# PierfrancescoArdino/C2M

Hardware: AMD Instinct MI355X
Metric: generator train-step frames/sec at 128x256x7 (higher is better)
Workload: dtype f32; 1 GPU; BASELINE configs[1]: 128x256, 7-frame clips (2 in + 5 predicted), batch 8/GPU, fp32, generator fwd+bwd only (no D), VGG loss on, random-init weights; global_batch=8, parallelism=single

## Files before the change

c2m_amd/csrc/conv_wino4.hip:

```cpp
#include "common.h"
#include <stdlib.h>

typedef float f32x16 __attribute__((ext_vector_type(16)));
typedef float f32x4 __attribute__((ext_vector_type(4)));
typedef float f32x2 __attribute__((ext_vector_type(2)));
typedef unsigned u32x4 __attribute__((ext_vector_type(4)));
#define W4_OOB 0x80000000u

struct Wino4P {
    const float* U;
    const float* X;
    float* Y;
    const float* bias;
    float* Y2;
    long y2_sn, y2_sc, y2_sh;
    int lo_y, lo_x, ext_y, ext_x;
    int M, K, nimg;
    int Hi, Wi, Ho, Wo;
    int iy0, ix0;
    int reflect;
    long in_sn, out_sn, out_sc, out_sh, out_off;
    int in_sc, in_sh;
    unsigned x_bytes;
    int nchunks, mtiles;
    int act;
    float slope;
    const float* R;
    int r_l;
};

#if !defined(W4_SKEW) && !defined(W4_FUSED)
#define W4_FUSED 1
#endif

constexpr int W4_CK = 8;
constexpr int W4_TH = 4, W4_TW = 8;
constexpr int W4_OR = 4 * W4_TH, W4_OC = 4 * W4_TW;
constexpr int W4_PH = W4_OR + 2, W4_PW = W4_OC + 2;
constexpr int W4_PITCH = 40;
constexpr int W4_PPOS = W4_PH * W4_PITCH;
constexpr int W4_ROWS = (W4_PPOS + 63) / 64;
constexpr int W4_PCS = 722;
constexpr int W4_PBUF = W4_CK * W4_PCS + 48;
constexpr int W4_TAB = W4_ROWS * 64;
constexpr int W4_VBUF = 36 * W4_CK * 32;

#define W4_BT(o0, o1, o2, o3, o4, o5, x0, x1, x2, x3, x4, x5) \
    do {                                                      \
        const float a_ = (x4) - 2.25f * (x2), b_ = 0.75f * (x3) - 1.6875f * (x1);          \
        const float c_ = (x4) - 0.5625f * (x2), e_ = 1.5f * (x3) - 0.84375f * (x1);        \
        o0 = 1.265625f * (x0) - 2.8125f * (x2) + (x4);        \
        o1 = a_ + b_; o2 = a_ - b_; o3 = c_ + e_; o4 = c_ - e_; \
        o5 = 1.265625f * (x1) - 2.8125f * (x3) + (x5);        \
    } while (0)

#ifdef W4_TRACE
__device__ unsigned long long w4_trace_buf[8 * 16 * 4 + 8 * 2];
#define W4_STAMP(i) do { if (blockIdx.x == 0 && lane == 0 && n < 16) sTr[(wave * 16 + n) * 4 + (i)] = clock64(); } while (0)
C2M_API int c2m_wino4_trace_read(unsigned long long* host) {
    return (int)hipMemcpyFromSymbol(host, HIP_SYMBOL(w4_trace_buf), sizeof(w4_trace_buf));
}
#else
#define W4_STAMP(i) do { } while (0)
#endif

__global__ __launch_bounds__(512, 2) void conv_wino4_kernel(const Wino4P p) {
    __shared__ __attribute__((aligned(16))) float smem[3 * W4_PBUF + W4_TAB + 2 * W4_VBUF];
#ifdef W4_TRACE
    __shared__ unsigned long long sTr[8 * 16 * 4 + 8 * 2];
    const unsigned long long t_begin = clock64();
#endif
#define sP (smem)
#define sVo (reinterpret_cast<unsigned*>(smem + 3 * W4_PBUF))
#define sV (smem + 3 * W4_PBUF + W4_TAB)
    const int tid = threadIdx.x, lane = tid & 63;
    const int wave = __builtin_amdgcn_readfirstlane(tid >> 6);
    const int wm = wave & 1, fg = wave >> 1;
    const bool t_first = (wave ^ (wave >> 2)) & 1;
    const int regions_x = (p.Wo + W4_OC - 1) / W4_OC, regions_y = (p.Ho + W4_OR - 1) / W4_OR;
    int rb, mt;
    {
        const unsigned L = blockIdx.x, total = gridDim.x;
        const unsigned q = total >> 3, r = total & 7u, x = L & 7u, j = L >> 3;
        const unsigned w = x * q + (x < r ? x : r) + j;
        mt = (int)(w % (unsigned)p.mtiles); rb = (int)(w / (unsigned)p.mtiles);
    }
    const int rx = rb % regions_x; rb /= regions_x;
    const int ry = rb % regions_y; const int img = rb / regions_y;
    const int oy0 = ry * W4_OR, ox0 = rx * W4_OC;
    const int nchunks = p.nchunks;

    {
        const unsigned img_byte = (unsigned)(img * (int)p.in_sn) * 4u;
        for (int pos = tid; pos < W4_TAB; pos += 512) {
            const int r = pos / W4_PITCH, c = pos % W4_PITCH;
            int iy = oy0 + p.iy0 + r, ix = ox0 + p.ix0 + c;
            if (p.reflect) {
                iy = iy < 0 ? -iy : iy; iy = iy >= p.Hi ? 2 * p.Hi - 2 - iy : iy;
                ix = ix < 0 ? -ix : ix; ix = ix >= p.Wi ? 2 * p.Wi - 2 - ix : ix;
            }
            const bool ok = pos < W4_PPOS && c < W4_PW && (unsigned)iy < (unsigned)p.Hi && (unsigned)ix < (unsigned)p.Wi;
            sVo[pos] = ok ? img_byte + (unsigned)(iy * p.in_sh + ix) * 4u : W4_OOB;
        }
    }
    __syncthreads();

    const unsigned long xaddr = (unsigned long)p.X;
    const u32x4 rs = {(unsigned)xaddr, (unsigned)(xaddr >> 32) & 0xffffu, p.x_bytes, 0x00020000u};
    const unsigned sp_lds = (unsigned)(unsigned long)(__attribute__((address_space(3))) float*)&smem[0];
    unsigned pvo[W4_ROWS];
#pragma unroll
    for (int dr = 0; dr < W4_ROWS; ++dr) pvo[dr] = sVo[dr * 64 + lane];
    auto load_patch = [&](int chunk, int buf, const int dr0 = 0, const int dr1 = W4_ROWS) __attribute__((always_inline)) {
#ifdef W4_ZERO_RECORDS
        const int ch = chunk * W4_CK + wave;
        u32x4 rsk = rs;
        rsk[2] = (chunk < nchunks && ch < p.K) ? p.x_bytes : 0u;
#else
        int ch = chunk * W4_CK + wave;
        ch = ch < p.K ? ch : p.K - 1;
        const u32x4 rsk = rs;
#endif
        const int soff = ch * p.in_sc * 4;
#pragma unroll
        for (int dr = dr0; dr < dr1; ++dr) {
            const unsigned vo = pvo[dr];
            const unsigned dst = sp_lds + (unsigned)((buf * W4_PBUF + wave * W4_PCS + dr * 64) * 4);
            if (dr * 64 + 64 <= W4_PPOS || dr * 64 + lane < W4_PPOS)
                asm volatile("s_mov_b32 m0, %0\n\ts_nop 0\n\tbuffer_load_dword %1, %2, %3 offen lds"
                             :: "s"(dst), "v"(vo), "s"(rsk), "s"(soff) : "memory");
        }
    };
    const unsigned long uaddr = (unsigned long)p.U;
    const u32x4 urs = {(unsigned)uaddr, (unsigned)(uaddr >> 32) & 0xffffu, 0xffffffffu, 0x00020000u};
    const unsigned uvo = (unsigned)((((mt * 8 + wave) * 9) * 64 + lane) * 16);
    const unsigned ustride_b = (unsigned)p.mtiles * 8u * 9u * 64u * 16u;
    f32x4 ua[9];
    auto load_u = [&](int chunk) __attribute__((always_inline)) {
        const int s0 = (int)((unsigned)(chunk < nchunks ? chunk : 0) * ustride_b), s1 = s0 + 4096, s2 = s0 + 8192;
#pragma unroll
        for (int f = 0; f < 9; ++f)
            asm volatile("buffer_load_dwordx4 %0, %1, %2, %3 offen offset:%4"
                         : "=&v"(ua[f]) : "v"(uvo), "s"(urs), "s"(f < 4 ? s0 : (f < 8 ? s1 : s2)), "n"((f & 3) * 1024) : "memory");
    };

    f32x16 acc[9];
#pragma unroll
    for (int f = 0; f < 9; ++f)
#pragma unroll
        for (int r = 0; r < 16; ++r) acc[f][r] = 0.f;

    const int item = tid & 255, th = __builtin_amdgcn_readfirstlane(tid >> 8);
    const int tk = item >> 5, tn = item & 31;
    const int pbase = tk * W4_PCS + (4 * (tn >> 3)) * W4_PITCH + 4 * (tn & 7);
    auto transform = [&](int pb, int vb) __attribute__((always_inline)) {
        const float* __restrict__ src = sP + pb * W4_PBUF + pbase;
        float t[3][6];
#pragma unroll
        for (int cp = 0; cp < 3; ++cp) {
            f32x2 d[6];
#pragma unroll
            for (int r = 0; r < 6; ++r) d[r] = *reinterpret_cast<const f32x2*>(src + r * W4_PITCH + 2 * cp);
#pragma unroll
            for (int e = 0; e < 2; ++e) {
                const float d0 = d[0][e], d1 = d[1][e], d2 = d[2][e], d3 = d[3][e], d4 = d[4][e], d5 = d[5][e];
                const int c = 2 * cp + e;
                if (th == 0) {
                    const float a_ = d4 - 2.25f * d2, b_ = 0.75f * d3 - 1.6875f * d1;
                    t[0][c] = 1.265625f * d0 - 2.8125f * d2 + d4; t[1][c] = a_ + b_; t[2][c] = a_ - b_;
                } else {
                    const float c_ = d4 - 0.5625f * d2, e_ = 1.5f * d3 - 0.84375f * d1;
                    t[0][c] = c_ + e_; t[1][c] = c_ - e_; t[2][c] = 1.265625f * d1 - 2.8125f * d3 + d5;
                }
            }
        }
        float* __restrict__ v = sV + vb * W4_VBUF + tk * 32 + tn;
#pragma unroll
        for (int a = 0; a < 3; ++a) {
            float o0, o1, o2, o3, o4, o5;
            W4_BT(o0, o1, o2, o3, o4, o5, t[a][0], t[a][1], t[a][2], t[a][3], t[a][4], t[a][5]);
            const int xi0 = 6 * (3 * th + a);
            v[(xi0 + 0) * W4_CK * 32] = o0; v[(xi0 + 1) * W4_CK * 32] = o1; v[(xi0 + 2) * W4_CK * 32] = o2;
            v[(xi0 + 3) * W4_CK * 32] = o3; v[(xi0 + 4) * W4_CK * 32] = o4; v[(xi0 + 5) * W4_CK * 32] = o5;
            __builtin_amdgcn_sched_barrier(0);
        }
    };
    auto mma = [&](int cur, int next_chunk) __attribute__((always_inline)) {
        const float* __restrict__ vb = sV + cur * W4_VBUF + (9 * fg * W4_CK + (lane >> 5)) * 32 + (lane & 31);
        const int s0 = (int)((unsigned)(next_chunk < nchunks ? next_chunk : 0) * ustride_b), s1 = s0 + 4096, s2 = s0 + 8192;
#pragma unroll
        for (int g3 = 0; g3 < 3; ++g3) {
            float b[3][4];
#pragma unroll
            for (int f = 0; f < 3; ++f)
#pragma unroll
                for (int kk = 0; kk < 4; ++kk) b[f][kk] = vb[((3 * g3 + f) * W4_CK + 2 * kk) * 32];
#pragma unroll
            for (int kk = 0; kk < 4; ++kk)
#pragma unroll
                for (int f = 0; f < 3; ++f) {
                    const f32x4 u = ua[3 * g3 + f];
                    const float av = kk == 0 ? u.x : (kk == 1 ? u.y : (kk == 2 ? u.z : u.w));
                    acc[3 * g3 + f] = __builtin_amdgcn_mfma_f32_32x32x2f32(av, b[f][kk], acc[3 * g3 + f], 0, 0, 0);
                }
            __builtin_amdgcn_sched_barrier(0);
#pragma unroll
            for (int f = 3 * g3; f < 3 * g3 + 3; ++f)
                asm volatile("buffer_load_dwordx4 %0, %1, %2, %3 offen offset:%4"
                             : "=&v"(ua[f]) : "v"(uvo), "s"(urs), "s"(f < 4 ? s0 : (f < 8 ? s1 : s2)), "n"((f & 3) * 1024) : "memory");
            __builtin_amdgcn_sched_barrier(0);
        }
    };

#ifdef W4_FUSED
    const float cA = th ? 0.5625f : 2.25f, cB3 = th ? 1.5f : 0.75f, cB1 = th ? 0.84375f : 1.6875f;
    const int xrow = th ? 5 : 0, r_single = th ? 5 : 0, r_plus = th ? 3 : 1, r_minus = th ? 4 : 2;
    auto fused = [&](int cur, int next_chunk, int pb, int dbuf) __attribute__((always_inline)) {
        const float* __restrict__ vb = sV + cur * W4_VBUF + (9 * fg * W4_CK + (lane >> 5)) * 32 + (lane & 31);
        const float* __restrict__ src = sP + pb * W4_PBUF + pbase;
        const int s0 = (int)((unsigned)(next_chunk < nchunks ? next_chunk : 0) * ustride_b), s1 = s0 + 4096, s2 = s0 + 8192;
        float ts[6], tp[6], tm[6];
        float b[3][4];
        f32x2 d1, d2, d3, d4, dx;
        auto reads = [&](const int g3) __attribute__((always_inline)) {
#pragma unroll
            for (int f = 0; f < 3; ++f)
#pragma unroll
                for (int kk = 0; kk < 4; ++kk) b[f][kk] = vb[((3 * g3 + f) * W4_CK + 2 * kk) * 32];
            d1 = *reinterpret_cast<const f32x2*>(src + 1 * W4_PITCH + 2 * g3); d2 = *reinterpret_cast<const f32x2*>(src + 2 * W4_PITCH + 2 * g3);
            d3 = *reinterpret_cast<const f32x2*>(src + 3 * W4_PITCH + 2 * g3); d4 = *reinterpret_cast<const f32x2*>(src + 4 * W4_PITCH + 2 * g3);
            dx = *reinterpret_cast<const f32x2*>(src + xrow * W4_PITCH + 2 * g3);
        };
        asm volatile("s_waitcnt vmcnt(12)" ::: "memory");
#pragma unroll
        for (int f = 0; f < 3; ++f) asm volatile("" : "+v"(ua[f]));
        reads(0);
#pragma unroll
        for (int g3 = 0; g3 < 3; ++g3) {
#pragma unroll
            for (int kk = 0; kk < 4; ++kk)
#pragma unroll
                for (int f = 0; f < 3; ++f) {
                    const f32x4 u = ua[3 * g3 + f];
                    const float av = kk == 0 ? u.x : (kk == 1 ? u.y : (kk == 2 ? u.z : u.w));
                    acc[3 * g3 + f] = __builtin_amdgcn_mfma_f32_32x32x2f32(av, b[f][kk], acc[3 * g3 + f], 0, 0, 0);
                }
#pragma unroll
            for (int e = 0; e < 2; ++e) {
                const int c = 2 * g3 + e;
                const float q0 = th ? d1[e] : dx[e], q2 = th ? d3[e] : d2[e], q4 = th ? dx[e] : d4[e];
                ts[c] = 1.265625f * q0 - 2.8125f * q2 + q4;
                const float a_ = d4[e] - cA * d2[e], b_ = cB3 * d3[e] - cB1 * d1[e];
                tp[c] = a_ + b_; tm[c] = a_ - b_;
            }
            if (g3 == 0) __builtin_amdgcn_sched_group_barrier(0x100, 17, 0);
#pragma unroll
            for (int q = 0; q < 12; ++q) {
                __builtin_amdgcn_sched_group_barrier(0x008, 1, 0);
                __builtin_amdgcn_sched_group_barrier(0x002, 2, 0);
            }
            __builtin_amdgcn_sched_barrier(0);
            if (g3 < 2) reads(g3 + 1);
            if (g3 < 2) load_patch(next_chunk + 1, dbuf, 6 * g3, 6 * g3 + 6);
#pragma unroll
            for (int f = 3 * g3; f < 3 * g3 + 3; ++f)
                asm volatile("buffer_load_dwordx4 %0, %1, %2, %3 offen offset:%4"
                             : "=&v"(ua[f]) : "v"(uvo), "s"(urs), "s"(f < 4 ? s0 : (f < 8 ? s1 : s2)), "n"((f & 3) * 1024) : "memory");
            if (g3 == 0) asm volatile("s_waitcnt vmcnt(12)" ::: "memory");
            if (g3 == 1) asm volatile("s_waitcnt vmcnt(18)" ::: "memory");
            if (g3 < 2) {
#pragma unroll
                for (int f = 3 * g3 + 3; f < 3 * g3 + 6; ++f) asm volatile("" : "+v"(ua[f]));
            }
            __builtin_amdgcn_sched_barrier(0);
        }
        float* __restrict__ v = sV + (cur ^ 1) * W4_VBUF + tk * 32 + tn;
#pragma unroll
        for (int a = 0; a < 3; ++a) {
            const float* t = a == 0 ? ts : (a == 1 ? tp : tm);
            const int row = a == 0 ? r_single : (a == 1 ? r_plus : r_minus);
            float o0, o1, o2, o3, o4, o5;
            W4_BT(o0, o1, o2, o3, o4, o5, t[0], t[1], t[2], t[3], t[4], t[5]);
            float* __restrict__ vr = v + 6 * row * W4_CK * 32;
            vr[0] = o0; vr[1 * W4_CK * 32] = o1; vr[2 * W4_CK * 32] = o2;
            vr[3 * W4_CK * 32] = o3; vr[4 * W4_CK * 32] = o4; vr[5 * W4_CK * 32] = o5;
        }
    };
#endif

    load_patch(0, 0);
    load_patch(1, 1);
    load_u(0);
    asm volatile("s_waitcnt vmcnt(21)" ::: "memory");
    __syncthreads();
    transform(0, 0);
#ifdef W4_FUSED
    asm volatile("s_waitcnt vmcnt(0)" ::: "memory");
#else
    asm volatile("s_waitcnt vmcnt(9)" ::: "memory");
#endif
    int pn = 1;
#ifdef W4_PRIO
    if (wave >= 4) __builtin_amdgcn_s_setprio(1);
#endif
    for (int n = 0; n < nchunks; ++n) {
        __syncthreads();
        W4_STAMP(0);
        const int cur = n & 1;
        const int dbuf = pn == 2 ? 0 : pn + 1;
#ifndef W4_FUSED
        load_patch(n + 2, dbuf);
#endif
        __builtin_amdgcn_sched_barrier(0);
#ifdef W4_FUSED
        W4_STAMP(1);
        fused(cur, n + 1, pn, dbuf);
        W4_STAMP(2);
        W4_STAMP(3);
#else
        if (t_first) transform(pn, cur ^ 1);
        asm volatile("s_waitcnt vmcnt(12)" ::: "memory");
#pragma unroll
        for (int f = 0; f < 9; ++f) asm volatile("" : "+v"(ua[f]));
        W4_STAMP(1);
        mma(cur, n + 1);
        W4_STAMP(2);
        if (!t_first) transform(pn, cur ^ 1);
        W4_STAMP(3);
#endif
#ifdef W4_FUSED
        asm volatile("s_waitcnt vmcnt(6)" ::: "memory");
#else
        asm volatile("s_waitcnt vmcnt(9)" ::: "memory");
#endif
        pn = pn == 2 ? 0 : pn + 1;
    }
    asm volatile("s_waitcnt vmcnt(0)" ::: "memory");
#pragma unroll
    for (int f = 0; f < 9; ++f) asm volatile("" :: "v"(ua[f]));
    __syncthreads();

    float* __restrict__ sR = sV;
    const int etile = tid & 31, ecl = tid >> 5;
    const int ety = etile >> 3, etx = etile & 7;
    const int oyb = oy0 + 4 * ety, oxb = ox0 + 4 * etx;
    float bias4[4];
#pragma unroll
    for (int pass = 0; pass < 4; ++pass) {
        const int co = mt * 64 + (pass >> 1) * 32 + (pass & 1) * 16 + ecl;
        bias4[pass] = (p.bias && co < p.M) ? p.bias[co] : 0.f;
    }
#pragma unroll
    for (int pass = 0; pass < 4; ++pass) {
        const int pwm = pass >> 1, hf = pass & 1;
        __syncthreads();
        if (wm == pwm) {
#pragma unroll
            for (int f = 0; f < 9; ++f)
#pragma unroll
                for (int rr = 0; rr < 8; ++rr) {
                    const int rowl = (rr & 3) + 8 * (rr >> 2) + 4 * (lane >> 5);
                    sR[((9 * fg + f) * 16 + rowl) * 32 + (lane & 31)] = hf ? acc[f][8 + rr] : acc[f][rr];
                }
        }
        __syncthreads();
        const int cout = mt * 64 + pwm * 32 + hf * 16 + ecl;
        float y[4][4];
        {
            float s[6][4];
#pragma unroll
            for (int i = 0; i < 6; ++i) {
                const float* __restrict__ q = sR + ((6 * i) * 16 + ecl) * 32 + etile;
                const float m0 = q[0], m1 = q[16 * 32], m2 = q[2 * 16 * 32], m3 = q[3 * 16 * 32], m4 = q[4 * 16 * 32], m5 = q[5 * 16 * 32];
                const float pp = m1 + m2, nn = m1 - m2, PP = m3 + m4, NN = m3 - m4;
                s[i][0] = m0 + pp + PP; s[i][1] = 0.75f * nn + 1.5f * NN; s[i][2] = 0.5625f * pp + 2.25f * PP;
                s[i][3] = 0.421875f * nn + 3.375f * NN + m5;
            }
#pragma unroll
            for (int c = 0; c < 4; ++c) {
                const float pp = s[1][c] + s[2][c], nn = s[1][c] - s[2][c], PP = s[3][c] + s[4][c], NN = s[3][c] - s[4][c];
                y[0][c] = s[0][c] + pp + PP; y[1][c] = 0.75f * nn + 1.5f * NN; y[2][c] = 0.5625f * pp + 2.25f * PP;
                y[3][c] = 0.421875f * nn + 3.375f * NN + s[5][c];
            }
        }
        if (cout < p.M) {
            const float bb = bias4[pass];
            const float* __restrict__ rb = p.R ? p.R + ((long)img * p.M + cout) * 4 * p.r_l : nullptr;
#pragma unroll
            for (int r = 0; r < 4; ++r) {
                const int oy = oyb + r;
                if (oy >= p.Ho) continue;
                if (rb) {
                    if (oy == 1 || oy == p.Ho - 2) {
                        const float* __restrict__ rr = rb + (oy == 1 ? 0 : p.r_l) + oxb;
#pragma unroll
                        for (int c = 0; c < 4; ++c) if (oxb + c < p.Wo) y[r][c] += rr[c];
                    }
                    if (oxb <= 1 && oxb + 3 >= 1) {
                        const float v = rb[2 * p.r_l + oy];
#pragma unroll
                        for (int c = 0; c < 4; ++c) if (oxb + c == 1) y[r][c] += v;
                    }
                    if (oxb <= p.Wo - 2 && oxb + 3 >= p.Wo - 2) {
                        const float v = rb[3 * p.r_l + oy];
#pragma unroll
                        for (int c = 0; c < 4; ++c) if (oxb + c == p.Wo - 2) y[r][c] += v;
                    }
                }
                if (p.act == C2M_ACT_NONE) {
#pragma unroll
                    for (int c = 0; c < 4; ++c) y[r][c] += bb;
                } else if (p.act == C2M_ACT_LRELU) {
#pragma unroll
                    for (int c = 0; c < 4; ++c) { const float v = y[r][c] + bb; y[r][c] = v > 0.f ? v : p.slope * v; }
                } else {
#pragma unroll
                    for (int c = 0; c < 4; ++c) y[r][c] = c2m_act(y[r][c] + bb, p.act, p.slope);
                }
                float* __restrict__ yb0 = p.Y + p.out_off + (long)img * p.out_sn + (long)cout * p.out_sc + (long)oy * p.out_sh + oxb;
                typedef float f32x4u __attribute__((ext_vector_type(4), aligned(4)));
                const f32x4u vv = {y[r][0], y[r][1], y[r][2], y[r][3]};
                const int yi = oy - p.lo_y, xi0 = oxb - p.lo_x;
                const bool row_in = p.Y2 && (unsigned)yi < (unsigned)p.ext_y;
                const bool all_in = row_in && xi0 >= 0 && xi0 + 3 < p.ext_x;
                const bool all_out = !row_in || xi0 + 3 < 0 || xi0 >= p.ext_x;
                if (oxb + 3 < p.Wo && (!p.Y2 || all_out)) {
                    *reinterpret_cast<f32x4u*>(yb0) = vv;
                } else if (oxb + 3 < p.Wo && all_in) {
                    *reinterpret_cast<f32x4u*>(p.Y2 + (long)img * p.y2_sn + (long)cout * p.y2_sc + (long)yi * p.y2_sh + xi0) = vv;
                } else {
#pragma unroll
                    for (int c = 0; c < 4; ++c) {
                        if (oxb + c >= p.Wo) continue;
                        const int xi = oxb + c - p.lo_x;
                        if (row_in && (unsigned)xi < (unsigned)p.ext_x)
                            p.Y2[(long)img * p.y2_sn + (long)cout * p.y2_sc + (long)yi * p.y2_sh + xi] = y[r][c];
                        else
                            yb0[c] = y[r][c];
                    }
                }
            }
        }
    }
#ifdef W4_TRACE
    if (blockIdx.x == 0 && lane == 0) { sTr[8 * 16 * 4 + wave * 2] = t_begin; sTr[8 * 16 * 4 + wave * 2 + 1] = clock64(); }
    __syncthreads();
    if (blockIdx.x == 0)
        for (int i = tid; i < 8 * 16 * 4 + 8 * 2; i += 512) w4_trace_buf[i] = sTr[i];
#endif
}

#undef sP
#undef sVo
#undef sV

__global__ void wino4_filter_kernel(const float* __restrict__ w, float* __restrict__ up, int M, int K, int Cin_native,
                                    int dgrad, int mtiles, long pairs) {
    for (long i = blockIdx.x * (long)blockDim.x + threadIdx.x; i < pairs; i += (long)gridDim.x * blockDim.x) {
        const int kk = (int)(i & 3); long r = i >> 2;
        const int lane = (int)(r & 63); r >>= 6;
        const int wm = (int)(r & 1); r >>= 1;
        const int mt = (int)(r % mtiles); const int chunk = (int)(r / mtiles);
        const int m = mt * 64 + wm * 32 + (lane & 31), c = chunk * W4_CK + 2 * kk + (lane >> 5);
        float u[6][6];
#pragma unroll
        for (int a = 0; a < 6; ++a)
#pragma unroll
            for (int b2 = 0; b2 < 6; ++b2) u[a][b2] = 0.f;
        if (m < M && c < K) {
            const float* __restrict__ g = dgrad ? w + ((long)c * Cin_native + m) * 9 : w + ((long)m * Cin_native + c) * 9;
            float gg[3][3];
#pragma unroll
            for (int a = 0; a < 3; ++a)
#pragma unroll
                for (int b2 = 0; b2 < 3; ++b2) gg[a][b2] = dgrad ? g[(2 - a) * 3 + (2 - b2)] : g[a * 3 + b2];
            float row[6][3];
#pragma unroll
            for (int b2 = 0; b2 < 3; ++b2) {
                const float g0 = gg[0][b2], g1 = gg[1][b2], g2 = gg[2][b2];
                row[0][b2] = (64.f / 81.f) * g0;
                row[1][b2] = -(128.f / 243.f) * g0 - (32.f / 81.f) * g1 - (8.f / 27.f) * g2;
                row[2][b2] = -(128.f / 243.f) * g0 + (32.f / 81.f) * g1 - (8.f / 27.f) * g2;
                row[3][b2] = (32.f / 243.f) * g0 + (16.f / 81.f) * g1 + (8.f / 27.f) * g2;
                row[4][b2] = (32.f / 243.f) * g0 - (16.f / 81.f) * g1 + (8.f / 27.f) * g2;
                row[5][b2] = g2;
            }
#pragma unroll
            for (int a = 0; a < 6; ++a) {
                const float r0 = row[a][0], r1 = row[a][1], r2 = row[a][2];
                u[a][0] = (64.f / 81.f) * r0;
                u[a][1] = -(128.f / 243.f) * r0 - (32.f / 81.f) * r1 - (8.f / 27.f) * r2;
                u[a][2] = -(128.f / 243.f) * r0 + (32.f / 81.f) * r1 - (8.f / 27.f) * r2;
                u[a][3] = (32.f / 243.f) * r0 + (16.f / 81.f) * r1 + (8.f / 27.f) * r2;
                u[a][4] = (32.f / 243.f) * r0 - (16.f / 81.f) * r1 + (8.f / 27.f) * r2;
                u[a][5] = r2;
            }
        }
        const long base = ((long)chunk * mtiles + mt) * 8;
#pragma unroll
        for (int a = 0; a < 6; ++a)
#pragma unroll
            for (int b2 = 0; b2 < 6; ++b2) {
                const int xi = 6 * a + b2, fgi = xi / 9, f = xi % 9;
                up[((((base + ((fgi << 1) | wm)) * 9 + f) * 64 + lane) << 2) + kk] = u[a][b2];
            }
    }
}

C2M_API long c2m_wino4_upack_floats(int M, int K) {
    return 36L * (c2m_cdiv(M, 64) * 64L) * (c2m_cdiv(K, W4_CK) * (long)W4_CK);
}

C2M_API int c2m_wino4_filter_transform(const float* w, float* upack, int Cout, int Cin, int dgrad, void* stream) {
    C2M_ENTER();
    const int M = dgrad ? Cin : Cout, K = dgrad ? Cout : Cin;
    if (M <= 0 || K <= 0) return 0;
    const long total = c2m_wino4_upack_floats(M, K);
    if (total * 4 >= 0xffffffffL) return (int)hipErrorInvalidValue;
    hipLaunchKernelGGL(wino4_filter_kernel, dim3(c2m_grid(total / 36, 256)), dim3(256), 0, (hipStream_t)stream, w, upack, M,
                       K, Cin, dgrad, c2m_cdiv(M, 64), total / 36);
    return (int)hipGetLastError();
}

C2M_API int c2m_wino4_regions(int Ho, int Wo) { return c2m_cdiv(Ho, W4_OR) * c2m_cdiv(Wo, W4_OC); }

C2M_API int c2m_conv_wino4(const float* upack, const float* X, float* Y, float* Y_interior, const float* bias,
                           const int64_t* g, int act, float slope, void* stream) {
    C2M_ENTER();
    Wino4P p;
    p.U = upack; p.X = X; p.Y = Y; p.bias = bias;
    p.Y2 = Y_interior; p.y2_sn = p.y2_sc = p.y2_sh = 0; p.lo_y = p.lo_x = p.ext_y = p.ext_x = 0;
    if (Y_interior) {
        p.y2_sn = g[C2M_WG_Y2_SN]; p.y2_sc = g[C2M_WG_Y2_SC]; p.y2_sh = g[C2M_WG_Y2_SH];
        p.lo_y = (int)g[C2M_WG_LO_Y]; p.lo_x = (int)g[C2M_WG_LO_X]; p.ext_y = (int)g[C2M_WG_EXT_Y]; p.ext_x = (int)g[C2M_WG_EXT_X];
    }
    p.M = (int)g[C2M_WG_M]; p.K = (int)g[C2M_WG_K]; p.nimg = (int)g[C2M_WG_NIMG];
    p.Hi = (int)g[C2M_WG_HI]; p.Wi = (int)g[C2M_WG_WI]; p.Ho = (int)g[C2M_WG_HO]; p.Wo = (int)g[C2M_WG_WO];
    p.iy0 = (int)g[C2M_WG_IY0]; p.ix0 = (int)g[C2M_WG_IX0]; p.reflect = (int)g[C2M_WG_REFLECT];
    p.in_sn = g[C2M_WG_IN_SN]; p.in_sc = (int)g[C2M_WG_IN_SC]; p.in_sh = (int)g[C2M_WG_IN_SH];
    p.out_sn = g[C2M_WG_OUT_SN]; p.out_sc = g[C2M_WG_OUT_SC]; p.out_sh = g[C2M_WG_OUT_SH]; p.out_off = g[C2M_WG_OUT_OFF];
    if (g[C2M_WG_X_BYTES] <= 0 || g[C2M_WG_X_BYTES] >= 0x80000000LL) return (int)hipErrorInvalidValue;
    p.x_bytes = (unsigned)g[C2M_WG_X_BYTES];
    if (g[C2M_WG_NKT] != 0 || g[C2M_WG_PTAB] != 0) return (int)hipErrorInvalidValue;
    p.R = (const float*)(uintptr_t)g[C2M_WG_RING]; p.r_l = (int)g[C2M_WG_RING_L];
    if (p.R && (Y_interior || p.reflect || p.Ho < 4 || p.Wo < 4 || p.r_l < p.Ho || p.r_l < p.Wo || p.out_off != 0)) return (int)hipErrorInvalidValue;
    p.act = act; p.slope = slope;
    if (p.M <= 0 || p.K <= 0 || p.nimg <= 0 || p.Ho <= 0 || p.Wo <= 0) return 0;
    if ((((uintptr_t)upack) & 15) != 0) return (int)hipErrorInvalidValue;
    p.nchunks = c2m_cdiv(p.K, W4_CK);
    p.mtiles = c2m_cdiv(p.M, 64);
    if (c2m_wino4_upack_floats(p.M, p.K) * 4 >= 0xffffffffL) return (int)hipErrorInvalidValue;
    const long regions = (long)p.nimg * c2m_wino4_regions(p.Ho, p.Wo);
    if (regions * p.mtiles > 0x7fffffffL) return (int)hipErrorInvalidValue;
    hipLaunchKernelGGL(conv_wino4_kernel, dim3((unsigned)(regions * p.mtiles)), dim3(512), 0, (hipStream_t)stream, p);
    return (int)hipGetLastError();
}
```

Measured before the change: 892.9 frames/s.

## Make Winograd conv kernel persistent with cross-tile prefetch overlapping epilogue

```diff
diff --git a/c2m_amd/csrc/conv_wino4.hip b/c2m_amd/csrc/conv_wino4.hip
--- a/c2m_amd/csrc/conv_wino4.hip
+++ b/c2m_amd/csrc/conv_wino4.hip
@@ -23,6 +23,7 @@
     int in_sc, in_sh;
     unsigned x_bytes;
     int nchunks, mtiles;
+    unsigned items;
     int act;
     float slope;
     const float* R;
@@ -56,7 +57,7 @@
 
 #ifdef W4_TRACE
 __device__ unsigned long long w4_trace_buf[8 * 16 * 4 + 8 * 2];
-#define W4_STAMP(i) do { if (blockIdx.x == 0 && lane == 0 && n < 16) sTr[(wave * 16 + n) * 4 + (i)] = clock64(); } while (0)
+#define W4_STAMP(i) do { if (blockIdx.x == 0 && lane == 0 && n < 16 && it == it_first) sTr[(wave * 16 + n) * 4 + (i)] = clock64(); } while (0)
 C2M_API int c2m_wino4_trace_read(unsigned long long* host) {
     return (int)hipMemcpyFromSymbol(host, HIP_SYMBOL(w4_trace_buf), sizeof(w4_trace_buf));
 }
@@ -65,7 +66,7 @@
 #endif
 
 __global__ __launch_bounds__(512, 2) void conv_wino4_kernel(const Wino4P p) {
-    __shared__ __attribute__((aligned(16))) float smem[3 * W4_PBUF + W4_TAB + 2 * W4_VBUF];
+    __shared__ __attribute__((aligned(16))) float smem[3 * W4_PBUF + W4_TAB + 2 * W4_VBUF + 64];
 #ifdef W4_TRACE
     __shared__ unsigned long long sTr[8 * 16 * 4 + 8 * 2];
     const unsigned long long t_begin = clock64();
@@ -73,28 +74,42 @@
 #define sP (smem)
 #define sVo (reinterpret_cast<unsigned*>(smem + 3 * W4_PBUF))
 #define sV (smem + 3 * W4_PBUF + W4_TAB)
+#define sBias (smem + 3 * W4_PBUF + W4_TAB + 2 * W4_VBUF)
     const int tid = threadIdx.x, lane = tid & 63;
     const int wave = __builtin_amdgcn_readfirstlane(tid >> 6);
     const int wm = wave & 1, fg = wave >> 1;
     const bool t_first = (wave ^ (wave >> 2)) & 1;
     const int regions_x = (p.Wo + W4_OC - 1) / W4_OC, regions_y = (p.Ho + W4_OR - 1) / W4_OR;
-    int rb, mt;
+    unsigned it, it_end;
     {
-        const unsigned L = blockIdx.x, total = gridDim.x;
-        const unsigned q = total >> 3, r = total & 7u, x = L & 7u, j = L >> 3;
-        const unsigned w = x * q + (x < r ? x : r) + j;
-        mt = (int)(w % (unsigned)p.mtiles); rb = (int)(w / (unsigned)p.mtiles);
+        const unsigned L = blockIdx.x, G = gridDim.x;
+        const unsigned q = p.items >> 3, r = p.items & 7u, x = L & 7u, j = L >> 3;
+        const unsigned sx = x * q + (x < r ? x : r), cx = q + (x < r ? 1u : 0u);
+        const unsigned gx = (G >> 3) + (x < (G & 7u) ? 1u : 0u);
+        it = sx + (unsigned)((unsigned long)j * cx / gx);
+        it_end = sx + (unsigned)((unsigned long)(j + 1) * cx / gx);
     }
-    const int rx = rb % regions_x; rb /= regions_x;
-    const int ry = rb % regions_y; const int img = rb / regions_y;
-    const int oy0 = ry * W4_OR, ox0 = rx * W4_OC;
+    if (it >= it_end) return;
+#ifdef W4_TRACE
+    const unsigned it_first = it;
+#endif
+    struct Item { int mt, rb, img, oy0, ox0; };
+    auto decode = [&](unsigned w) __attribute__((always_inline)) {
+        Item d;
+        d.mt = (int)(w % (unsigned)p.mtiles); d.rb = (int)(w / (unsigned)p.mtiles);
+        const int rx = d.rb % regions_x, t = d.rb / regions_x;
+        d.img = t / regions_y;
+        d.oy0 = (t % regions_y) * W4_OR; d.ox0 = rx * W4_OC;
+        return d;
+    };
+    Item cur_it = decode(it);
     const int nchunks = p.nchunks;
 
-    {
-        const unsigned img_byte = (unsigned)(img * (int)p.in_sn) * 4u;
+    auto build_table = [&](const Item& d) __attribute__((always_inline)) {
+        const unsigned img_byte = (unsigned)(d.img * (int)p.in_sn) * 4u;
         for (int pos = tid; pos < W4_TAB; pos += 512) {
             const int r = pos / W4_PITCH, c = pos % W4_PITCH;
-            int iy = oy0 + p.iy0 + r, ix = ox0 + p.ix0 + c;
+            int iy = d.oy0 + p.iy0 + r, ix = d.ox0 + p.ix0 + c;
             if (p.reflect) {
                 iy = iy < 0 ? -iy : iy; iy = iy >= p.Hi ? 2 * p.Hi - 2 - iy : iy;
                 ix = ix < 0 ? -ix : ix; ix = ix >= p.Wi ? 2 * p.Wi - 2 - ix : ix;
@@ -102,15 +117,23 @@
             const bool ok = pos < W4_PPOS && c < W4_PW && (unsigned)iy < (unsigned)p.Hi && (unsigned)ix < (unsigned)p.Wi;
             sVo[pos] = ok ? img_byte + (unsigned)(iy * p.in_sh + ix) * 4u : W4_OOB;
         }
-    }
+    };
+    auto stage_bias = [&](int mt_) __attribute__((always_inline)) {
+        if (tid < 64) { const int co = mt_ * 64 + tid; sBias[tid] = (p.bias && co < p.M) ? p.bias[co] : 0.f; }
+    };
+    build_table(cur_it);
+    stage_bias(cur_it.mt);
     __syncthreads();
 
     const unsigned long xaddr = (unsigned long)p.X;
     const u32x4 rs = {(unsigned)xaddr, (unsigned)(xaddr >> 32) & 0xffffu, p.x_bytes, 0x00020000u};
     const unsigned sp_lds = (unsigned)(unsigned long)(__attribute__((address_space(3))) float*)&smem[0];
     unsigned pvo[W4_ROWS];
-#pragma unroll
-    for (int dr = 0; dr < W4_ROWS; ++dr) pvo[dr] = sVo[dr * 64 + lane];
+    auto read_pvo = [&]() __attribute__((always_inline)) {
+#pragma unroll
+        for (int dr = 0; dr < W4_ROWS; ++dr) pvo[dr] = sVo[dr * 64 + lane];
+    };
+    read_pvo();
     auto load_patch = [&](int chunk, int buf, const int dr0 = 0, const int dr1 = W4_ROWS) __attribute__((always_inline)) {
 #ifdef W4_ZERO_RECORDS
         const int ch = chunk * W4_CK + wave;
@@ -133,7 +156,7 @@
     };
     const unsigned long uaddr = (unsigned long)p.U;
     const u32x4 urs = {(unsigned)uaddr, (unsigned)(uaddr >> 32) & 0xffffu, 0xffffffffu, 0x00020000u};
-    const unsigned uvo = (unsigned)((((mt * 8 + wave) * 9) * 64 + lane) * 16);
+    unsigned uvo = (unsigned)((((cur_it.mt * 8 + wave) * 9) * 64 + lane) * 16);
     const unsigned ustride_b = (unsigned)p.mtiles * 8u * 9u * 64u * 16u;
     f32x4 ua[9];
     auto load_u = [&](int chunk) __attribute__((always_inline)) {
@@ -145,10 +168,6 @@
     };
 
     f32x16 acc[9];
-#pragma unroll
-    for (int f = 0; f < 9; ++f)
-#pragma unroll
-        for (int r = 0; r < 16; ++r) acc[f][r] = 0.f;
 
     const int item = tid & 255, th = __builtin_amdgcn_readfirstlane(tid >> 8);
     const int tk = item >> 5, tn = item & 31;
@@ -299,10 +318,16 @@
 #else
     asm volatile("s_waitcnt vmcnt(9)" ::: "memory");
 #endif
-    int pn = 1;
 #ifdef W4_PRIO
     if (wave >= 4) __builtin_amdgcn_s_setprio(1);
 #endif
+    for (;;) {
+    const int mt = cur_it.mt, img = cur_it.img, oy0 = cur_it.oy0, ox0 = cur_it.ox0;
+#pragma unroll
+    for (int f = 0; f < 9; ++f)
+#pragma unroll
+        for (int r = 0; r < 16; ++r) acc[f][r] = 0.f;
+    int pn = 1;
     for (int n = 0; n < nchunks; ++n) {
         __syncthreads();
         W4_STAMP(0);
@@ -340,16 +365,29 @@
     for (int f = 0; f < 9; ++f) asm volatile("" :: "v"(ua[f]));
     __syncthreads();
 
+    const bool more = it + 1 < it_end;
+    Item nxt = cur_it;
+    if (more) {
+        nxt = decode(it + 1);
+        if (nxt.rb != cur_it.rb) {
+            build_table(nxt);
+            __syncthreads();
+            read_pvo();
+        }
+        load_patch(0, 0);
+        load_patch(1, 1);
+    }
+
     float* __restrict__ sR = sV;
-    const int etile = tid & 31, ecl = tid >> 5;
+    const Wino4P& pe = p;
+    int etid = tid;
+    asm volatile("" : "+v"(etid));
+    const int etile = etid & 31, ecl = etid >> 5;
     const int ety = etile >> 3, etx = etile & 7;
     const int oyb = oy0 + 4 * ety, oxb = ox0 + 4 * etx;
     float bias4[4];
 #pragma unroll
-    for (int pass = 0; pass < 4; ++pass) {
-        const int co = mt * 64 + (pass >> 1) * 32 + (pass & 1) * 16 + ecl;
-        bias4[pass] = (p.bias && co < p.M) ? p.bias[co] : 0.f;
-    }
+    for (int pass = 0; pass < 4; ++pass) bias4[pass] = sBias[(pass >> 1) * 32 + (pass & 1) * 16 + ecl];
 #pragma unroll
     for (int pass = 0; pass < 4; ++pass) {
         const int pwm = pass >> 1, hf = pass & 1;
@@ -364,6 +402,11 @@
                 }
         }
         __syncthreads();
+        if (pass == 3 && more) {
+            uvo = (unsigned)((((nxt.mt * 8 + wave) * 9) * 64 + lane) * 16);
+            stage_bias(nxt.mt);
+            load_u(0);
+        }
         const int cout = mt * 64 + pwm * 32 + hf * 16 + ecl;
         float y[4][4];
         {
@@ -383,64 +426,75 @@
                 y[3][c] = 0.421875f * nn + 3.375f * NN + s[5][c];
             }
         }
-        if (cout < p.M) {
+        if (pass == 3 && more) {
+            asm volatile("s_waitcnt vmcnt(0)" ::: "memory");
+#pragma unroll
+            for (int f = 0; f < 9; ++f) asm volatile("" : "+v"(ua[f]));
+            __syncthreads();
+            read_pvo();
+            transform(0, 0);
+        }
+        if (cout < pe.M) {
             const float bb = bias4[pass];
-            const float* __restrict__ rb = p.R ? p.R + ((long)img * p.M + cout) * 4 * p.r_l : nullptr;
+            const float* __restrict__ rb = pe.R ? pe.R + ((long)img * pe.M + cout) * 4 * pe.r_l : nullptr;
 #pragma unroll
             for (int r = 0; r < 4; ++r) {
                 const int oy = oyb + r;
-                if (oy >= p.Ho) continue;
+                if (oy >= pe.Ho) continue;
                 if (rb) {
-                    if (oy == 1 || oy == p.Ho - 2) {
-                        const float* __restrict__ rr = rb + (oy == 1 ? 0 : p.r_l) + oxb;
-#pragma unroll
-                        for (int c = 0; c < 4; ++c) if (oxb + c < p.Wo) y[r][c] += rr[c];
+                    if (oy == 1 || oy == pe.Ho - 2) {
+                        const float* __restrict__ rr = rb + (oy == 1 ? 0 : pe.r_l) + oxb;
+#pragma unroll
+                        for (int c = 0; c < 4; ++c) if (oxb + c < pe.Wo) y[r][c] += rr[c];
                     }
                     if (oxb <= 1 && oxb + 3 >= 1) {
-                        const float v = rb[2 * p.r_l + oy];
+                        const float v = rb[2 * pe.r_l + oy];
 #pragma unroll
                         for (int c = 0; c < 4; ++c) if (oxb + c == 1) y[r][c] += v;
                     }
-                    if (oxb <= p.Wo - 2 && oxb + 3 >= p.Wo - 2) {
-                        const float v = rb[3 * p.r_l + oy];
-#pragma unroll
-                        for (int c = 0; c < 4; ++c) if (oxb + c == p.Wo - 2) y[r][c] += v;
+                    if (oxb <= pe.Wo - 2 && oxb + 3 >= pe.Wo - 2) {
+                        const float v = rb[3 * pe.r_l + oy];
+#pragma unroll
+                        for (int c = 0; c < 4; ++c) if (oxb + c == pe.Wo - 2) y[r][c] += v;
                     }
                 }
-                if (p.act == C2M_ACT_NONE) {
+                if (pe.act == C2M_ACT_NONE) {
 #pragma unroll
                     for (int c = 0; c < 4; ++c) y[r][c] += bb;
-                } else if (p.act == C2M_ACT_LRELU) {
-#pragma unroll
-                    for (int c = 0; c < 4; ++c) { const float v = y[r][c] + bb; y[r][c] = v > 0.f ? v : p.slope * v; }
+                } else if (pe.act == C2M_ACT_LRELU) {
+#pragma unroll
+                    for (int c = 0; c < 4; ++c) { const float v = y[r][c] + bb; y[r][c] = v > 0.f ? v : pe.slope * v; }
                 } else {
 #pragma unroll
-                    for (int c = 0; c < 4; ++c) y[r][c] = c2m_act(y[r][c] + bb, p.act, p.slope);
+                    for (int c = 0; c < 4; ++c) y[r][c] = c2m_act(y[r][c] + bb, pe.act, pe.slope);
                 }
-                float* __restrict__ yb0 = p.Y + p.out_off + (long)img * p.out_sn + (long)cout * p.out_sc + (long)oy * p.out_sh + oxb;
+                float* __restrict__ yb0 = pe.Y + pe.out_off + (long)img * pe.out_sn + (long)cout * pe.out_sc + (long)oy * pe.out_sh + oxb;
                 typedef float f32x4u __attribute__((ext_vector_type(4), aligned(4)));
                 const f32x4u vv = {y[r][0], y[r][1], y[r][2], y[r][3]};
-                const int yi = oy - p.lo_y, xi0 = oxb - p.lo_x;
-                const bool row_in = p.Y2 && (unsigned)yi < (unsigned)p.ext_y;
-                const bool all_in = row_in && xi0 >= 0 && xi0 + 3 < p.ext_x;
-                const bool all_out = !row_in || xi0 + 3 < 0 || xi0 >= p.ext_x;
-                if (oxb + 3 < p.Wo && (!p.Y2 || all_out)) {
+                const int yi = oy - pe.lo_y, xi0 = oxb - pe.lo_x;
+                const bool row_in = pe.Y2 && (unsigned)yi < (unsigned)pe.ext_y;
+                const bool all_in = row_in && xi0 >= 0 && xi0 + 3 < pe.ext_x;
+                const bool all_out = !row_in || xi0 + 3 < 0 || xi0 >= pe.ext_x;
+                if (oxb + 3 < pe.Wo && (!pe.Y2 || all_out)) {
                     *reinterpret_cast<f32x4u*>(yb0) = vv;
-                } else if (oxb + 3 < p.Wo && all_in) {
-                    *reinterpret_cast<f32x4u*>(p.Y2 + (long)img * p.y2_sn + (long)cout * p.y2_sc + (long)yi * p.y2_sh + xi0) = vv;
+                } else if (oxb + 3 < pe.Wo && all_in) {
+                    *reinterpret_cast<f32x4u*>(pe.Y2 + (long)img * pe.y2_sn + (long)cout * pe.y2_sc + (long)yi * pe.y2_sh + xi0) = vv;
                 } else {
 #pragma unroll
                     for (int c = 0; c < 4; ++c) {
-                        if (oxb + c >= p.Wo) continue;
-                        const int xi = oxb + c - p.lo_x;
-                        if (row_in && (unsigned)xi < (unsigned)p.ext_x)
-                            p.Y2[(long)img * p.y2_sn + (long)cout * p.y2_sc + (long)yi * p.y2_sh + xi] = y[r][c];
+                        if (oxb + c >= pe.Wo) continue;
+                        const int xi = oxb + c - pe.lo_x;
+                        if (row_in && (unsigned)xi < (unsigned)pe.ext_x)
+                            pe.Y2[(long)img * pe.y2_sn + (long)cout * pe.y2_sc + (long)yi * pe.y2_sh + xi] = y[r][c];
                         else
                             yb0[c] = y[r][c];
                     }
                 }
             }
         }
+    }
+    if (!more) break;
+    cur_it = nxt; ++it;
     }
 #ifdef W4_TRACE
     if (blockIdx.x == 0 && lane == 0) { sTr[8 * 16 * 4 + wave * 2] = t_begin; sTr[8 * 16 * 4 + wave * 2 + 1] = clock64(); }
@@ -453,6 +507,7 @@
 #undef sP
 #undef sVo
 #undef sV
+#undef sBias
 
 __global__ void wino4_filter_kernel(const float* __restrict__ w, float* __restrict__ up, int M, int K, int Cin_native,
                                     int dgrad, int mtiles, long pairs) {
@@ -523,6 +578,17 @@
 }
 
 C2M_API int c2m_wino4_regions(int Ho, int Wo) { return c2m_cdiv(Ho, W4_OR) * c2m_cdiv(Wo, W4_OC); }
+
+static int wino4_cu_count() {
+    static int cached[64];
+    int dev = 0;
+    if (hipGetDevice(&dev) != hipSuccess || dev < 0) return 0;
+    if (dev < 64 && cached[dev] > 0) return cached[dev];
+    int n = 0;
+    if (hipDeviceGetAttribute(&n, hipDeviceAttributeMultiprocessorCount, dev) != hipSuccess) return 0;
+    if (dev < 64) cached[dev] = n;
+    return n;
+}
 
 C2M_API int c2m_conv_wino4(const float* upack, const float* X, float* Y, float* Y_interior, const float* bias,
                            const int64_t* g, int act, float slope, void* stream) {
@@ -552,6 +618,10 @@
     if (c2m_wino4_upack_floats(p.M, p.K) * 4 >= 0xffffffffL) return (int)hipErrorInvalidValue;
     const long regions = (long)p.nimg * c2m_wino4_regions(p.Ho, p.Wo);
     if (regions * p.mtiles > 0x7fffffffL) return (int)hipErrorInvalidValue;
-    hipLaunchKernelGGL(conv_wino4_kernel, dim3((unsigned)(regions * p.mtiles)), dim3(512), 0, (hipStream_t)stream, p);
+    p.items = (unsigned)(regions * p.mtiles);
+    const int cus = wino4_cu_count();
+    if (cus <= 0) return (int)hipErrorInvalidDevice;
+    const unsigned grid = p.items < (unsigned)cus ? p.items : (unsigned)cus;
+    hipLaunchKernelGGL(conv_wino4_kernel, dim3(grid), dim3(512), 0, (hipStream_t)stream, p);
     return (int)hipGetLastError();
 }
```

After: 845.0 frames/s. -5.4%, worse.
